# jiahuei/sparse-image-captioning

Hardware: AMD Instinct MI355X
Metric: captions/sec (higher is better)
Workload: dtype bf16; 1 GPU; configs[1]: ORT dense, 256 images x 5 captions, teacher-forcing XE fwd+bwd+clip+Adam; images_per_gpu=256, regions=36, captions_per_image=5, parallelism=single

## Files before the change

include/ortk.h:

```cpp
#ifndef ORTK_H
#define ORTK_H

#include <stddef.h>
#include <stdint.h>

#ifdef __cplusplus
extern "C" {
#endif

#define ORTK_VERSION 4
#define ORTK_EINVAL (-1)
#define ORTK_ENOSPC (-2)
#define ORTK_ENOSYS (-3)
#define ORTK_EEXCHANGE (-4)

typedef void* ortk_stream;

int ortk_version(void);
int ortk_device_ok(void);

struct ortk_sparse_plan;
typedef struct ortk_config {
    int32_t d_model, d_ff, n_layers, n_heads;
    int32_t vocab, feat, seq_len;
    int32_t pad_id, bos_id, eos_id, unk_id;
// ... 128 lines not shown
    int32_t attn16_min_lq;
    int32_t side_stream;
    int32_t row_chain;
    int32_t chain_wide;
    int32_t spmm_alias;
    int32_t f32_split;
    int32_t wgrad_wgs;
    int32_t wgrad_group;
    int32_t wgrad_group_splitk;
    int32_t wgrad_group_wgs;
    int32_t wgrad_group_tail;
    int32_t feats_bf16;
    int32_t ln_fuse;
    int32_t samp_epilogue;
    int32_t gemm_epilogue;
} ortk_tuning;
void ortk_get_tuning(ortk_tuning* out);
int ortk_set_tuning(const ortk_tuning* t);

#define ORTK_DEC_UNFUSED 1
#define ORTK_DEC_STACK 2
#define ORTK_DEC_SPARSE_STREAM 4
#define ORTK_DEC_STACK_RB20 8
#define ORTK_DEC_STACK_SPLIT 16
#define ORTK_DEC_SPLIT_SMALL 32
#define ORTK_DEC_SPARSE_GATHER 64
typedef struct ortk_decode_opts {
    int32_t beam_size;
    int32_t num_random_sample;
    float   temperature;
// ... 102 lines not shown
    float drop_p; uint32_t drop_seed;
    const float* d_o; void* dq; void* d_k; void* dv; float* dscore;
    int64_t lddo, lddq, lddk, lddv;
    int32_t o_dtype, dqkv_dtype;
    int32_t kv_dtype;
    const float* k_new; const float* v_new; int64_t ld_new;
    int32_t bwd_part;
    int32_t precision;
    int32_t qkv_dtype;
    const int32_t* q_off; int32_t q_off_stride; int32_t kv_ragged;
    int32_t drop_tf_T, drop_tf_t, drop_tf_lk;
    const int32_t* drop_rows;
} ortk_attn_args;
int ortk_attention_fwd(const ortk_attn_args* a, ortk_stream stream);
int ortk_attention_bwd(const ortk_attn_args* a, ortk_stream stream);

int ortk_embed_fwd(const int64_t* seq, int64_t seq_stride, const float* lut, const float* pe, float* out, float* keymask,
                   int64_t R, int32_t T, int32_t t0, int32_t d, int32_t pad_id, float drop_p, uint32_t seed, ortk_stream stream);
int ortk_embed_bwd(const int64_t* seq, int64_t seq_stride, const float* dout, float* dlut,
                   int64_t R, int32_t T, int32_t d, float drop_p, uint32_t seed, ortk_stream stream);

int ortk_log_softmax(float* x, int64_t rows, int32_t V, int64_t ld, float scale, ortk_stream stream);
int64_t ortk_xent_scratch_floats(int64_t rows);
int ortk_xent_fwd_bwd(const float* logits, const int64_t* targets, int64_t target_stride, int32_t T, const float* weight,
                      const float* norm_dev, float* loss_dev, float* row_loss, int64_t rows, int32_t V, int64_t ld,
                      void* dlogits, int32_t dl_dtype, int64_t ld_dl, ortk_stream stream);
int ortk_log_softmax_bwd(const float* logp, const float* dlogp, int64_t ld_in, void* dlogits, int32_t dl_dtype,
                         int64_t ld_out, int64_t rows, int32_t V, ortk_stream stream);

int ortk_colsum(const void* x, int32_t x_dtype, int64_t ld, float* out, int64_t M, int32_t N, ortk_stream stream);
// ... 39 lines not shown
```

sparse-image-captioning_amd/_lib.py:

```python
import ctypes as C
import os

import torch

_HERE = os.path.dirname(os.path.abspath(__file__))
LIB_PATH = os.path.join(_HERE, "libortk.so")


class OrtkUnavailable(RuntimeError):
    pass


class OrtkError(RuntimeError):
    pass


class Config(C.Structure):
    _fields_ = [("d_model", C.c_int32), ("d_ff", C.c_int32), ("n_layers", C.c_int32), ("n_heads", C.c_int32),
                ("vocab", C.c_int32), ("feat", C.c_int32), ("seq_len", C.c_int32),
                ("pad_id", C.c_int32), ("bos_id", C.c_int32), ("eos_id", C.c_int32), ("unk_id", C.c_int32),
                ("box_trig", C.c_int32), ("precision", C.c_int32), ("drop_src", C.c_float), ("drop", C.c_float),
                ("share_enc", C.c_int32 * 16), ("share_dec", C.c_int32 * 16),
                ("share_att_enc", C.c_int32), ("share_att_dec", C.c_int32), ("no_box", C.c_int32),
                ("sparse_fwd", C.c_void_p), ("sparse_bwd", C.c_void_p)]
# ... 57 lines not shown
                ("n2", C.c_int32), ("out2", C.c_void_p), ("drop_p", C.c_float), ("eps", C.c_float), ("drop_rows", C.c_void_p)]


class MaskedAdamArgs(C.Structure):
    _fields_ = [("w", C.c_void_p), ("g", C.c_void_p), ("mw", C.c_void_p), ("vw", C.c_void_p),
                ("ml", C.c_void_p), ("mm", C.c_void_p), ("mv", C.c_void_p),
                ("draws", C.c_void_p), ("active", C.c_void_p), ("extra_coef", C.c_void_p),
                ("n", C.c_int64), ("index0", C.c_int64), ("mode", C.c_int32), ("seed", C.c_uint32),
                ("lr_w", C.c_float), ("eps_w", C.c_float), ("lr_m", C.c_float), ("eps_m", C.c_float),
                ("beta1", C.c_float), ("beta2", C.c_float), ("clip", C.c_float), ("bc1", C.c_float), ("bc2", C.c_float)]


class Tuning(C.Structure):
    _fields_ = [("gemm_t64", C.c_int32), ("attn_impl", C.c_int32), ("attn16_min_lq", C.c_int32),
                ("side_stream", C.c_int32), ("row_chain", C.c_int32), ("chain_wide", C.c_int32), ("spmm_alias", C.c_int32), ("f32_split", C.c_int32), ("wgrad_wgs", C.c_int32),
                ("wgrad_group", C.c_int32), ("wgrad_group_splitk", C.c_int32), ("wgrad_group_wgs", C.c_int32), ("wgrad_group_tail", C.c_int32), ("feats_bf16", C.c_int32), ("ln_fuse", C.c_int32), ("samp_epilogue", C.c_int32), ("gemm_epilogue", C.c_int32)]


DEC_UNFUSED, DEC_STACK, DEC_SPARSE_STREAM, DEC_STACK_RB20, DEC_STACK_SPLIT, DEC_SPLIT_SMALL, DEC_SPARSE_GATHER = 1, 2, 4, 8, 16, 32, 64


class DecodeOpts(C.Structure):
    _fields_ = [("beam_size", C.c_int32), ("num_random_sample", C.c_int32), ("temperature", C.c_float),
                ("decoding_constraint", C.c_int32), ("length_penalty", C.c_int32), ("length_alpha", C.c_double),
                ("seed", C.c_uint64), ("sparse", C.POINTER(EllPlanStruct)), ("exec_flags", C.c_int32), ("with_greedy", C.c_int32), ("sample_row_offset", C.c_int64),
                ("train", C.c_int32), ("drop_seed", C.c_uint64), ("memory", C.c_void_p)]


class GemmArgs(C.Structure):
    _fields_ = [("A", C.c_void_p), ("B", C.c_void_p), ("C", C.c_void_p),
                ("lda", C.c_int64), ("ldb", C.c_int64), ("ldc", C.c_int64),
# ... 78 lines not shown
    "ortk_prof_enable": (_I32, [_I32]),
    "ortk_prof_collect": (_I32, [_I32, C.POINTER(_I64), C.POINTER(C.c_double), C.POINTER(C.c_double)]),
    "ortk_prof_collect_bytes": (_I32, [_I32, C.POINTER(C.c_double)]),
    "ortk_prof_collect_units": (_I32, [_I32, C.POINTER(C.c_double)]),
    "ortk_layernorm_fwd": (_I32, [_P, _P, _P, _P, _I32, _P, _I64, _I32, _F, _P]),
    "ortk_layernorm_bwd": (_I32, [_P, _P, _P, _P, _P, _P, _P, _P, _I64, _I32, _F, _P]),
    "ortk_layernorm_bwd_drop": (_I32, [_P, _P, _P, _P, _P, _P, _P, _P, _I64, _I32, _F, _P, _I32, _F, C.c_uint32, _P]),
    "ortk_layernorm_bwd_drop_rows": (_I32, [_P, _P, _P, _P, _P, _P, _P, _P, _I64, _I32, _F, _P, _I32, _F, C.c_uint32, _P, _P]),
    "ortk_layernorm_bwd_dt": (_I32, [_P, _I32, _P, _P, _P, _P, _P, _P, _P, _I64, _I32, _F, _P, _I32, _F, C.c_uint32, _P, _P]),
    "ortk_box_logbias_fwd": (_I32, [_P, C.POINTER(_P), C.POINTER(_P), C.POINTER(_F), _P, _I32, _I32, _I32, _I32, _P]),
    "ortk_box_logbias_bwd": (_I32, [_P, C.POINTER(_P), C.POINTER(_P), C.POINTER(_F), _P, C.POINTER(_P), C.POINTER(_P),
                                   _I32, _I32, _I32, _I32, _P]),
    "ortk_box_embedding": (_I32, [_P, C.POINTER(_F), _P, _I32, _I32, _P]),
    "ortk_attention_fwd": (_I32, [C.POINTER(AttnArgs), _P]),
    "ortk_attention_bwd": (_I32, [C.POINTER(AttnArgs), _P]),
    "ortk_valid_position_tables": (_I32, [_P, _I32, _I32, _P, _P, _P]),
    "ortk_embed_fwd": (_I32, [_P, _I64, _P, _P, _P, _P, _I64, _I32, _I32, _I32, _I32, _F, _U32, _P]),
    "ortk_embed_bwd": (_I32, [_P, _I64, _P, _P, _I64, _I32, _I32, _F, _U32, _P]),
    "ortk_log_softmax": (_I32, [_P, _I64, _I32, _I64, _F, _P]),
    "ortk_xent_scratch_floats": (_I64, [_I64]),
    "ortk_xent_fwd_bwd": (_I32, [_P, _P, _I64, _I32, _P, _P, _P, _P, _I64, _I32, _I64, _P, _I32, _I64, _P]),
    "ortk_log_softmax_bwd": (_I32, [_P, _P, _I64, _P, _I32, _I64, _I64, _I32, _P]),
    "ortk_colsum": (_I32, [_P, _I32, _I64, _P, _I64, _I32, _P]),
    "ortk_gate_apply": (_I32, [_P, _P, _P, _I32, _I64, _F, _P]),
    "ortk_dropout_apply": (_I32, [_P, _P, _I32, _I64, _F, _U32, _P]),
    "ortk_dropout_apply_rows": (_I32, [_P, _P, _I32, _I64, _I32, _F, _U32, _P, _P]),
    "ortk_dropout_site_seed": (_U32, [_U64, _I32, _I32, _I32]),
    "ortk_cast_bf16": (_I32, [_P, _P, _I64, _P]),
    "ortk_fill": (_I32, [_P, _I64, _F, _P]),
    "ortk_sum_scratch_floats": (_I64, [_I64]),
# ... 4 lines not shown
    "ortk_mask_bwd": (_I32, [_P, _P, _P, _P, _P, _I64, _I32, _U32, _P, _P]),
    "ortk_masked_adam_step": (_I32, [C.POINTER(MaskedAdamArgs), _P]),
    "ortk_mask_count": (_I32, [_P, _I64, _I32, _P, _P]),
    "ortk_mask_apply_draws": (_I32, [_P, _P, _P, _P, _I64, _P]),
    "ortk_mask_bwd_draws": (_I32, [_P, _P, _P, _P, _P, _P, _I64, _P, _P]),
    "ortk_decode_step_workspace_bytes": (_SZ, [_CFG, _I32]),
    "ortk_project_memory": (_I32, [_CFG, _P, _P, _I64, _P, _SZ, _P, _P]),
    "ortk_decode_step": (_I32, [_CFG, _P, _P, _I32, _I32, _I32, _I32, _P, _P, _P, _P, _I32, _P, _SZ, _P, _I64, _P]),
    "ortk_axpy_cols": (_I32, [_P, _P, _I32, _I64, _I64, _I32, _P]),
    "ortk_linear_block": (_I32, [_CFG, _I32, C.POINTER(C.c_int64), C.POINTER(C.c_int32), C.POINTER(C.c_int32)]),
    "ortk_sparse_build": (_I32, [C.POINTER(EllPlanStruct), _P, _I32, _P]),
    "ortk_spmm": (_I32, [C.POINTER(EllPlanStruct), _I32, C.POINTER(SpmmArgs), _P]),
}

_lib = None
ABI_VERSION = 4


def lib():
    global _lib
    if _lib is None:
        if not os.path.exists(LIB_PATH):
            raise OrtkUnavailable(
                f"{LIB_PATH} is missing: build it with `python -c 'import __graft_entry__ as g; g.build()'` "
                "(or `make -C sparse-image-captioning_amd/csrc`).  There is no CPU / PyTorch fallback.")
        h = C.CDLL(LIB_PATH)
        h.ortk_version.restype = C.c_int32
        if h.ortk_version() != ABI_VERSION:
            raise OrtkUnavailable(
                f"{LIB_PATH} is ABI version {h.ortk_version()}, these bindings were written for version {ABI_VERSION} (include/ortk.h: "
                "ORTK_VERSION): a stale build.  Rebuild it with `make -C sparse-image-captioning_amd/csrc`.")
# ... 52 lines not shown
```

sparse-image-captioning_amd/csrc/ortk_attn.hip:

```cpp
#include <cstdlib>
#include "ortk_internal.h"

namespace {

constexpr int MAXK = 128;
constexpr int MAXD = 64;
constexpr int KP = MAXD + 1;

__device__ __forceinline__ float bcast(float v, int l) { return __shfl(v, l, 64); }

__device__ __forceinline__ void wave_sync() { __builtin_amdgcn_fence(__ATOMIC_ACQ_REL, "wavefront"); __builtin_amdgcn_wave_barrier(); }

struct Tiles {
    float (*k)[KP];
    float (*v)[KP];
    float* mask;
    float (*q)[MAXD];
    float (*p)[MAXK];
};
__host__ __device__ inline size_t fwd_lds_bytes(int Lk) {
    return sizeof(float) * ((size_t)2 * Lk * KP + MAXK + 4 * MAXD + 4 * MAXK);
}
__device__ __forceinline__ Tiles carve_fwd(float* base, int Lk) {
    Tiles t;
// ... 1007 lines not shown
    for (int64_t i = (int64_t)blockIdx.x * 256 + threadIdx.x; i < n; i += (int64_t)gridDim.x * 256) {
        const int64_t g = i / d; const int c = (int)(i - g * d);
        const int j = a.Lk - 1;
        const int64_t row = a.kv_index ? (int64_t)a.kv_index[g * a.Lk + j] : g * (a.kv_group_stride > 0 ? a.kv_group_stride : a.Lk) + j;
        st_elem(const_cast<float*>(a.k), row * a.ldk + c, a.kv_dtype, a.k_new[g * a.ld_new + c]);
        st_elem(const_cast<float*>(a.v), row * a.ldv + c, a.kv_dtype, a.v_new[g * a.ld_new + c]);
    }
}

static bool kv16_ok(const ortk_attn_args* a) {
    const bool rowdec = a->Lq == 1 && a->H == 8 && a->dk == 64 && a->Lk <= 32 && a->causal_period == 0 && a->drop_p == 0.f && !a->bias;
    const bool small = a->dk == 64 && a->Lq <= 16 && a->Lk <= 48 && !a->kv_index && (a->Lq >= 9 || a->Lk > 8) && !rowdec;
    return (rowdec || small) && a->ldk % 8 == 0 && a->ldv % 8 == 0 && attn_impl() == 0;
}

extern "C" int ortk_attention_fwd(const ortk_attn_args* a_in, ortk_stream stream) {
    if (int e = check(a_in)) return e;
    if (!a_in->o) return ORTK_EINVAL;
    if (a_in->nkv == 0) return 0;
    if (a_in->kv_dtype != 0 && (a_in->kv_dtype != 1 || !kv16_ok(a_in))) return ORTK_EINVAL;
    ortk_attn_args a_local = *a_in;
    ortk_attn_args* a = &a_local;
    if ((a->k_new != nullptr) != (a->v_new != nullptr)) return ORTK_EINVAL;
    if (a->k_new && (a->Lq != 1 || a->ld_new < (int64_t)a->H * a->dk)) return ORTK_EINVAL;
    if (a->k_new) {
        const bool rowdec = a->H == 8 && a->dk == 64 && a->Lk <= 32 && a->causal_period == 0 && a->drop_p == 0.f && !a->bias &&
                            a->ldq % 4 == 0 && a->ldk % 4 == 0 && a->ldv % 4 == 0 && a->ldo % 4 == 0 && a->ld_new % 4 == 0 && attn_impl() == 0 &&
                            ((reinterpret_cast<uintptr_t>(a->q) | reinterpret_cast<uintptr_t>(a->k) | reinterpret_cast<uintptr_t>(a->v) |
                              reinterpret_cast<uintptr_t>(a->o) | reinterpret_cast<uintptr_t>(a->k_new) | reinterpret_cast<uintptr_t>(a->v_new)) & 15) == 0;
        if (!rowdec) {
            const int64_t n = (int64_t)a->nkv * a->H * a->dk;
            hipLaunchKernelGGL(attn_kv_append_kernel, dim3((unsigned)std::max<int64_t>(1, std::min<int64_t>(ortk_cdiv(n, 256), 2048))), dim3(256), 0,
                               ortk_s(stream), *a);
            ORTK_CHECK_LAUNCH();
            a->k_new = a->v_new = nullptr;
        }
    }
    if ((attn_impl() == 0 || a->qkv_dtype) && ortk::attn16_ok(a, false)) return ortk::attn16_fwd(a, ortk_s(stream));
    if (a->qkv_dtype || a->q_off) return ORTK_EINVAL;
    ortk::lds_attr(reinterpret_cast<const void*>(attn_fwd_kernel), fwd_lds_bytes(MAXK));
    ortk::lds_attr(reinterpret_cast<const void*>(attn_fwd_wave_kernel), sizeof(float) * 4 * (2 * 64 * KP + 128));
    if (a->drop_tf_T > 0) {
        if (a->kv_dtype || a->qkv_dtype || a->Lk > MAXK || a->dk > MAXD) return ORTK_EINVAL;
        hipLaunchKernelGGL(attn_fwd_kernel, dim3((unsigned)(a->nkv * a->H)), dim3(256), fwd_lds_bytes(a->Lk), ortk_s(stream), *a);
        ORTK_CHECK_LAUNCH();
        return 0;
    }
    const bool use_mfma = attn_impl() == 0 ? a->Lq > 32 : attn_impl() == 3;
    const bool vec_kq = (a->ldk % 4 == 0) && (a->ldq % 4 == 0) && (a->dk % 4 == 0) &&
                        ((reinterpret_cast<uintptr_t>(a->k) | reinterpret_cast<uintptr_t>(a->q)) & 15) == 0;
    const bool al16 = ((reinterpret_cast<uintptr_t>(a->q) | reinterpret_cast<uintptr_t>(a->k) | reinterpret_cast<uintptr_t>(a->v) |
                        reinterpret_cast<uintptr_t>(a->o)) & 15) == 0;
// ... 35 lines not shown
        if (DKP == 64 && Lkp == 48)      hipLaunchKernelGGL((attn_fwd_mfma_kernel<48, 64>), mgrid, mblock, lds, ortk_s(stream), *a, Lkp, DKP);
        else if (DKP == 64 && Lkp == 32) hipLaunchKernelGGL((attn_fwd_mfma_kernel<32, 64>), mgrid, mblock, lds, ortk_s(stream), *a, Lkp, DKP);
        else if (DKP == 64 && Lkp == 64) hipLaunchKernelGGL((attn_fwd_mfma_kernel<64, 64>), mgrid, mblock, lds, ortk_s(stream), *a, Lkp, DKP);
        else                             hipLaunchKernelGGL((attn_fwd_mfma_kernel<0, 0>), mgrid, mblock, lds, ortk_s(stream), *a, Lkp, DKP);
    } else if (a->Lk <= 64 && attn_impl() == 1) {
        const int pairs = a->nkv * a->H;
        hipLaunchKernelGGL(attn_fwd_wave_kernel, dim3((unsigned)ortk_cdiv(pairs, 4)), dim3(256),
                           sizeof(float) * 4 * ((size_t)2 * a->Lk * KP + 128), ortk_s(stream), *a);
    } else {
        hipLaunchKernelGGL(attn_fwd_kernel, dim3((unsigned)(a->nkv * a->H)), dim3(256), fwd_lds_bytes(a->Lk), ortk_s(stream), *a);
    }
    ORTK_CHECK_LAUNCH();
    return 0;
}

extern "C" int ortk_attention_bwd(const ortk_attn_args* a, ortk_stream stream) {
    if (int e = check(a)) return e;
    if (a->kv_dtype != 0 || a->bwd_part < 0 || a->bwd_part > 2) return ORTK_EINVAL;
    if (!a->p || !a->d_o || !a->dq || !a->d_k || !a->dv || a->kv_index || a->kv_group_stride) return ORTK_EINVAL;
    if (a->nkv == 0) return 0;
    if ((attn_impl() == 0 || a->qkv_dtype) && ortk::attn16_ok(a, true))
        return a->bwd_part == 2 ? 0 : ortk::attn16_bwd(a, ortk_s(stream));
    if (a->qkv_dtype || a->q_off) return ORTK_EINVAL;
    ortk::lds_attr(reinterpret_cast<const void*>(attn_bwd_kernel), bwd_lds_bytes(MAXK));
    ortk::lds_attr(reinterpret_cast<const void*>(attn_bwd_wave_kernel<64>), sizeof(float) * 4 * (2 * 64 * KP + 192));
    ortk::lds_attr(reinterpret_cast<const void*>(attn_bwd_wave_kernel<48>), sizeof(float) * 4 * (2 * 48 * KP + 192));
    const int pairs = a->nkv * a->H;
    if (small_ok(a) && attn_impl() == 0 && a->ldv % 4 == 0 && a->lddo % 4 == 0 &&
        ((reinterpret_cast<uintptr_t>(a->v) | reinterpret_cast<uintptr_t>(a->d_o)) & 15) == 0) {
        const dim3 sgrid((unsigned)ortk_cdiv(pairs, 4));
        const int nit = a->Lq > 16 ? 2 : 1, njt = a->Lk > 16 ? 2 : 1;
        if (nit == 2 && njt == 2)      hipLaunchKernelGGL((attn_small_bwd_kernel<2, 2>), sgrid, dim3(256), 0, ortk_s(stream), *a);
        else if (nit == 2)             hipLaunchKernelGGL((attn_small_bwd_kernel<2, 1>), sgrid, dim3(256), 0, ortk_s(stream), *a);
        else if (njt == 2)             hipLaunchKernelGGL((attn_small_bwd_kernel<1, 2>), sgrid, dim3(256), 0, ortk_s(stream), *a);
        else                           hipLaunchKernelGGL((attn_small_bwd_kernel<1, 1>), sgrid, dim3(256), 0, ortk_s(stream), *a);
// ... 45 lines not shown
```

sparse-image-captioning_amd/csrc/ortk_internal.h:

```cpp
#pragma once
#include "ortk_common.h"

namespace ortk {

const ortk_tuning& tuning();
int lds_attr(const void* fn, size_t bytes);

bool ortk_prof_active();
bool ortk_prof_serial();
constexpr int PROF_KEY_DECSTACK = 16;
constexpr int PROF_KEY_CHAIN = 17;
constexpr int PROF_KEY_WGRAD_GROUP = 18;
struct ProfMark { hipEvent_t a, b; int key; double flops, bytes; bool live; int slot = -1; double per_count = 0.0; double units = 0.0 ; };
bool prof_begin(int key, double flops, double bytes, hipStream_t s, ProfMark& m);
void prof_end(const ProfMark& m, hipStream_t s);
unsigned long long* prof_slot(int* index);

int kv_append(const float* qkv, void* cache_k, void* cache_v, int32_t kv_dtype, int64_t rows, int32_t d, int32_t row_mult, int32_t tmax,
              int32_t t, hipStream_t s);

bool attn16_shape_ok(int Lq, int Lk, int dk);
bool attn16_ok(const ortk_attn_args* a, bool bwd);
int attn16_fwd(const ortk_attn_args* a, hipStream_t s);
int attn16_bwd(const ortk_attn_args* a, hipStream_t s);

struct WBlock { int32_t off, N, K, tile0; };
constexpr int MAX_WBLOCKS = 200;
struct WBlockTable { int32_t n, tiles; WBlock b[MAX_WBLOCKS]; };
int cast_bf16_transposed(const float* x, void* yt, const WBlockTable& t, hipStream_t s);

struct BeamState {
    int32_t B, b, L, V, eos;
    int64_t ldv;
    int32_t* seq[2];
    float* tok_lp[2];
    float* cum;
    int64_t* it;
    int32_t* kvidx[2];
    int32_t* done_seq;
// ... 126 lines not shown
```

sparse-image-captioning_amd/csrc/ortk_runtime.hip:

```cpp
#include <mutex>
#include <vector>
#include "ortk_internal.h"

namespace ortk {
static ortk_tuning tuning_defaults() {
    ortk_tuning t{};
    t.gemm_t64 = 640;
    t.attn_impl = 0;
    t.attn16_min_lq = 33;
    t.side_stream = 1;
    t.row_chain = 1;
    t.chain_wide = 1;
    t.spmm_alias = 1;
    t.f32_split = 1;
    t.wgrad_wgs = 384;
    t.wgrad_group = 3;
    t.wgrad_group_splitk = 0;
    t.wgrad_group_wgs = 80;
    t.wgrad_group_tail = 1;
    t.feats_bf16 = 1;
    t.ln_fuse = 0;
    t.samp_epilogue = 1;
    t.gemm_epilogue = 0;
    return t;
}
static ortk_tuning g_tuning = tuning_defaults();
const ortk_tuning& tuning() { return g_tuning; }
}

extern "C" void ortk_get_tuning(ortk_tuning* out) { if (out) *out = ortk::g_tuning; }
extern "C" int ortk_set_tuning(const ortk_tuning* t) {
    if (!t) return ORTK_EINVAL;
    auto in = [](int32_t v, int32_t lo, int32_t hi) { return v >= lo && v <= hi; };
    if (!in(t->attn_impl, 0, 4) || t->attn16_min_lq < 1 || !in(t->f32_split, 0, 7) || t->wgrad_wgs < 1 ||
        !in(t->wgrad_group, 0, 15) || !in(t->wgrad_group_splitk, 0, 8) || t->wgrad_group_wgs < 1 || !in(t->wgrad_group_tail, 0, 1) ||
        !in(t->feats_bf16, 0, 1) || !in(t->ln_fuse, 0, 15) || (t->ln_fuse & 2)  ||
        !in(t->samp_epilogue, 0, 1) || !in(t->gemm_epilogue, 0, 3)) return ORTK_EINVAL;
    ortk::g_tuning = *t;
    return 0;
}

namespace ortk {
int lds_attr(const void* fn, size_t bytes) {
    struct Key { int dev; const void* fn; size_t bytes; };
    static std::mutex mu;
    static std::vector<Key>* seen = new std::vector<Key>();
    int dev = 0;
    if (hipGetDevice(&dev) != hipSuccess) return ORTK_EINVAL;
    std::lock_guard<std::mutex> lk(mu);
    for (const Key& k : *seen) if (k.dev == dev && k.fn == fn && k.bytes >= bytes) return 0;
    if (hipFuncSetAttribute(fn, hipFuncAttributeMaxDynamicSharedMemorySize, (int)bytes) != hipSuccess) return ORTK_EINVAL;
    seen->push_back(Key{dev, fn, bytes});
// ... 91 lines not shown
```

Measured before the change: 132,200 captions/sec.

## Add whole-row MFMA attention kernels for short ragged caption sequences

```diff
diff --git a/include/ortk.h b/include/ortk.h
--- a/include/ortk.h
+++ b/include/ortk.h
@@ -8,7 +8,7 @@
 extern "C" {
 #endif
 
-#define ORTK_VERSION 4
+#define ORTK_VERSION 5
 #define ORTK_EINVAL (-1)
 #define ORTK_ENOSPC (-2)
 #define ORTK_ENOSYS (-3)
@@ -167,6 +167,7 @@
     int32_t ln_fuse;
     int32_t samp_epilogue;
     int32_t gemm_epilogue;
+    int32_t attn_rows;
 } ortk_tuning;
 void ortk_get_tuning(ortk_tuning* out);
 int ortk_set_tuning(const ortk_tuning* t);
@@ -299,6 +300,7 @@
 } ortk_attn_args;
 int ortk_attention_fwd(const ortk_attn_args* a, ortk_stream stream);
 int ortk_attention_bwd(const ortk_attn_args* a, ortk_stream stream);
+int ortk_attention_rows_serves(const ortk_attn_args* a, int bwd);
 
 int ortk_embed_fwd(const int64_t* seq, int64_t seq_stride, const float* lut, const float* pe, float* out, float* keymask,
                    int64_t R, int32_t T, int32_t t0, int32_t d, int32_t pad_id, float drop_p, uint32_t seed, ortk_stream stream);
diff --git a/scratch/attn_rows_bench.py b/scratch/attn_rows_bench.py
--- /dev/null
+++ b/scratch/attn_rows_bench.py
@@ -0,0 +1,55 @@
+import ctypes as C, os, statistics, sys
+sys.path[:0] = [os.path.join(os.path.dirname(os.path.abspath(__file__)), "..")]
+import torch
+import sparse_image_captioning_amd as P
+L = P._lib
+vals = [int(x) for x in sys.argv[1:] if "=" not in x] or [0, 1]
+for x in sys.argv[1:]:
+    if x.startswith("lib="):
+        L.LIB_PATH = x[4:]
+lib = L.lib()
+R, T, H, dk, NSET = 1280, 17, 8, 64, 4
+d = H * dk
+g = torch.Generator().manual_seed(0)
+lens = torch.randint(2, T + 1, (R,), generator=g)
+lens[:R // 2] = T
+while int(lens.sum()) > 16640:
+    i = int(torch.randint(R // 2, R, (1,), generator=g)); lens[i] = max(2, int(lens[i]) - 1)
+while int(lens.sum()) < 16640:
+    i = int(torch.randint(R // 2, R, (1,), generator=g)); lens[i] = min(T, int(lens[i]) + 1)
+off = torch.zeros(R + 1, dtype=torch.int32); off[1:] = lens.cumsum(0)
+M = int(off[-1])
+row_pos = torch.cat([c * T + torch.arange(int(n)) for c, n in enumerate(lens)]).int()
+sets = []
+for s in range(NSET):
+    t = dict(qkv=torch.randn(M, 3 * d, device="cuda").bfloat16(), do=torch.randn(M, d, device="cuda").bfloat16(),
+             o=torch.empty(M, d, device="cuda", dtype=torch.bfloat16), p=torch.empty(R, H, T, T, device="cuda"),
+             dqkv=torch.empty(M, 3 * d, device="cuda", dtype=torch.bfloat16), km=torch.ones(M, device="cuda"), off=off.cuda(), dr=row_pos.cuda())
+    a = L.AttnArgs()
+    a.precision = a.qkv_dtype = a.o_dtype = a.dqkv_dtype = 1
+    base, dbase = t["qkv"].data_ptr(), t["dqkv"].data_ptr()
+    a.q, a.k, a.v, a.o, a.p = base, base + 2 * d, base + 4 * d, t["o"].data_ptr(), t["p"].data_ptr()
+    a.ldq = a.ldk = a.ldv = a.lddq = a.lddk = a.lddv = 3 * d
+    a.ldo = a.lddo = d
+    a.d_o, a.dq, a.d_k, a.dv = t["do"].data_ptr(), dbase, dbase + 2 * d, dbase + 4 * d
+    a.nkv, a.H, a.Lq, a.Lk, a.dk, a.causal_period = R, H, T, T, dk, T
+    a.kmask, a.q_off, a.q_off_stride, a.kv_ragged, a.drop_rows = t["km"].data_ptr(), t["off"].data_ptr(), 1, 1, t["dr"].data_ptr()
+    a.drop_p, a.drop_seed = 0.1, 11
+    sets.append((a, t))
+print(f"{R} captions, {M} rows, lib {L.LIB_PATH}", flush=True)
+for v in vals:
+    L.set_tuning(attn_rows=v)
+    line = []
+    for name, fn in (("fwd", lib.ortk_attention_fwd), ("bwd", lib.ortk_attention_bwd)):
+        for a, _ in sets:
+            L.check(fn(C.byref(a), L.stream_ptr()), name)
+        torch.cuda.synchronize()
+        for _ in range(2):
+            ev = [(torch.cuda.Event(enable_timing=True), torch.cuda.Event(enable_timing=True)) for _ in range(24)]
+            for i, (e0, e1) in enumerate(ev):
+                e0.record(); fn(C.byref(sets[i % NSET][0]), L.stream_ptr()); e1.record()
+            torch.cuda.synchronize()
+            us = [e0.elapsed_time(e1) * 1e3 for e0, e1 in ev]
+            line.append(f"{name} {min(us):6.1f} / {statistics.median(us):6.1f}")
+    serves = [lib.ortk_attention_rows_serves(C.byref(sets[0][0]), b) for b in (0, 1)] if hasattr(lib, "ortk_attention_rows_serves") else "?"
+    print(f"attn_rows {v} (whole-row kernels serve fwd, bwd: {serves}):  " + "   ".join(line), flush=True)
diff --git a/sparse-image-captioning_amd/_lib.py b/sparse-image-captioning_amd/_lib.py
--- a/sparse-image-captioning_amd/_lib.py
+++ b/sparse-image-captioning_amd/_lib.py
@@ -95,7 +95,7 @@
 class Tuning(C.Structure):
     _fields_ = [("gemm_t64", C.c_int32), ("attn_impl", C.c_int32), ("attn16_min_lq", C.c_int32),
                 ("side_stream", C.c_int32), ("row_chain", C.c_int32), ("chain_wide", C.c_int32), ("spmm_alias", C.c_int32), ("f32_split", C.c_int32), ("wgrad_wgs", C.c_int32),
-                ("wgrad_group", C.c_int32), ("wgrad_group_splitk", C.c_int32), ("wgrad_group_wgs", C.c_int32), ("wgrad_group_tail", C.c_int32), ("feats_bf16", C.c_int32), ("ln_fuse", C.c_int32), ("samp_epilogue", C.c_int32), ("gemm_epilogue", C.c_int32)]
+                ("wgrad_group", C.c_int32), ("wgrad_group_splitk", C.c_int32), ("wgrad_group_wgs", C.c_int32), ("wgrad_group_tail", C.c_int32), ("feats_bf16", C.c_int32), ("ln_fuse", C.c_int32), ("samp_epilogue", C.c_int32), ("gemm_epilogue", C.c_int32), ("attn_rows", C.c_int32)]
 
 
 DEC_UNFUSED, DEC_STACK, DEC_SPARSE_STREAM, DEC_STACK_RB20, DEC_STACK_SPLIT, DEC_SPLIT_SMALL, DEC_SPARSE_GATHER = 1, 2, 4, 8, 16, 32, 64
@@ -204,6 +204,7 @@
     "ortk_box_embedding": (_I32, [_P, C.POINTER(_F), _P, _I32, _I32, _P]),
     "ortk_attention_fwd": (_I32, [C.POINTER(AttnArgs), _P]),
     "ortk_attention_bwd": (_I32, [C.POINTER(AttnArgs), _P]),
+    "ortk_attention_rows_serves": (_I32, [C.POINTER(AttnArgs), _I32]),
     "ortk_valid_position_tables": (_I32, [_P, _I32, _I32, _P, _P, _P]),
     "ortk_embed_fwd": (_I32, [_P, _I64, _P, _P, _P, _P, _I64, _I32, _I32, _I32, _I32, _F, _U32, _P]),
     "ortk_embed_bwd": (_I32, [_P, _I64, _P, _P, _I64, _I32, _I32, _F, _U32, _P]),
@@ -238,7 +239,7 @@
 }
 
 _lib = None
-ABI_VERSION = 4
+ABI_VERSION = 5
 
 
 def lib():
diff --git a/sparse-image-captioning_amd/csrc/ortk_attn.hip b/sparse-image-captioning_amd/csrc/ortk_attn.hip
--- a/sparse-image-captioning_amd/csrc/ortk_attn.hip
+++ b/sparse-image-captioning_amd/csrc/ortk_attn.hip
@@ -1045,6 +1045,8 @@
     return (rowdec || small) && a->ldk % 8 == 0 && a->ldv % 8 == 0 && attn_impl() == 0;
 }
 
+static bool rows_serves(const ortk_attn_args* a, bool bwd) { return (attn_impl() == 0 || a->qkv_dtype) && ortk::attn_rows_ok(a, bwd); }
+
 extern "C" int ortk_attention_fwd(const ortk_attn_args* a_in, ortk_stream stream) {
     if (int e = check(a_in)) return e;
     if (!a_in->o) return ORTK_EINVAL;
@@ -1067,6 +1069,7 @@
             a->k_new = a->v_new = nullptr;
         }
     }
+    if (rows_serves(a, false)) return ortk::attn_rows_fwd(a, ortk_s(stream));
     if ((attn_impl() == 0 || a->qkv_dtype) && ortk::attn16_ok(a, false)) return ortk::attn16_fwd(a, ortk_s(stream));
     if (a->qkv_dtype || a->q_off) return ORTK_EINVAL;
     ortk::lds_attr(reinterpret_cast<const void*>(attn_fwd_kernel), fwd_lds_bytes(MAXK));
@@ -1132,11 +1135,24 @@
     return 0;
 }
 
-extern "C" int ortk_attention_bwd(const ortk_attn_args* a, ortk_stream stream) {
+static int check_bwd(const ortk_attn_args* a) {
     if (int e = check(a)) return e;
     if (a->kv_dtype != 0 || a->bwd_part < 0 || a->bwd_part > 2) return ORTK_EINVAL;
     if (!a->p || !a->d_o || !a->dq || !a->d_k || !a->dv || a->kv_index || a->kv_group_stride) return ORTK_EINVAL;
+    return 0;
+}
+
+extern "C" int ortk_attention_rows_serves(const ortk_attn_args* a, int bwd) {
+    if (int e = bwd ? check_bwd(a) : check(a)) return e;
+    if (!bwd && !a->o) return ORTK_EINVAL;
+    return a->nkv > 0 && rows_serves(a, bwd != 0) ? 1 : 0;
+}
+
+extern "C" int ortk_attention_bwd(const ortk_attn_args* a, ortk_stream stream) {
+    if (int e = check_bwd(a)) return e;
     if (a->nkv == 0) return 0;
+    if (rows_serves(a, true))
+        return a->bwd_part == 2 ? 0 : ortk::attn_rows_bwd(a, ortk_s(stream));
     if ((attn_impl() == 0 || a->qkv_dtype) && ortk::attn16_ok(a, true))
         return a->bwd_part == 2 ? 0 : ortk::attn16_bwd(a, ortk_s(stream));
     if (a->qkv_dtype || a->q_off) return ORTK_EINVAL;
diff --git a/sparse-image-captioning_amd/csrc/ortk_attn_rows.hip b/sparse-image-captioning_amd/csrc/ortk_attn_rows.hip
--- /dev/null
+++ b/sparse-image-captioning_amd/csrc/ortk_attn_rows.hip
@@ -0,0 +1,439 @@
+#include <cstdlib>
+#include "ortk_internal.h"
+
+namespace {
+
+constexpr int PJ = 40;
+
+__device__ __forceinline__ void wsync() { __builtin_amdgcn_fence(__ATOMIC_ACQ_REL, "wavefront"); __builtin_amdgcn_wave_barrier(); }
+__device__ __forceinline__ bf16x4 cvt4(float4 v) { return (bf16x4){(__bf16)v.x, (__bf16)v.y, (__bf16)v.z, (__bf16)v.w}; }
+__device__ __forceinline__ bf16x4 cvt4(f32x4 v) { return (bf16x4){(__bf16)v[0], (__bf16)v[1], (__bf16)v[2], (__bf16)v[3]}; }
+__device__ __forceinline__ f32x4 mma(bf16x8 x, bf16x8 y, f32x4 acc) { return __builtin_amdgcn_mfma_f32_16x16x32_bf16(x, y, acc, 0, 0, 0); }
+
+template <int PITCH>
+__device__ __forceinline__ bf16x8 frag_row(const __bf16* img, int row, int k0) {
+    return *reinterpret_cast<const bf16x8*>(img + row * PITCH + k0);
+}
+template <int PITCH>
+__device__ __forceinline__ bf16x8 frag_tr(const __bf16* img, int x0, int lane, int zr) {
+    const int lr = lane & 15, lq = lane >> 4;
+    const int r0 = 8 * lq + (lr >> 2);
+    const int c = x0 + 4 * (lane & 3);
+    typedef bf16x4 __attribute__((address_space(3))) * lds4;
+    const bf16x4 lo = __builtin_amdgcn_ds_read_tr16_b64_v4bf16((lds4)(img + min(r0, zr) * PITCH + c));
+    const bf16x4 hi = __builtin_amdgcn_ds_read_tr16_b64_v4bf16((lds4)(img + min(r0 + 4, zr) * PITCH + c));
+    return (bf16x8){lo[0], lo[1], lo[2], lo[3], hi[0], hi[1], hi[2], hi[3]};
+}
+
+template <int DKT, int HW, int NU>
+__device__ __forceinline__ void span_load(bf16x8 (&v)[NU], const __bf16* src, int64_t ld, int rows, int nh, int tid) {
+    constexpr int CPH = DKT / 8, CPR = HW * CPH, NT = 64 * HW;
+#pragma unroll
+    for (int u = 0; u < NU; ++u) {
+        const int idx = tid + u * NT, r = idx / CPR, c = idx % CPR;
+        v[u] = (bf16x8){0, 0, 0, 0, 0, 0, 0, 0};
+        if (r < rows && c < nh * CPH) v[u] = *reinterpret_cast<const bf16x8*>(src + (int64_t)r * ld + c * 8);
+    }
+}
+template <int DKT, int HW, int NU>
+__device__ __forceinline__ void span_store(const bf16x8 (&v)[NU], __bf16* img, int rows_img, int tid) {
+    constexpr int CPH = DKT / 8, CPR = HW * CPH, NT = 64 * HW, PD = DKT + 8;
+#pragma unroll
+    for (int u = 0; u < NU; ++u) {
+        const int idx = tid + u * NT, r = idx / CPR, c = idx % CPR;
+        if (r < rows_img) *reinterpret_cast<bf16x8*>(img + ((c / CPH) * rows_img + r) * PD + (c % CPH) * 8) = v[u];
+    }
+}
+template <int DKT, int HW>
+__device__ __forceinline__ void span_out(__bf16* dst, int64_t ld, const __bf16* img, int rows_img, int rows, int nh, int tid) {
+    constexpr int CPH = DKT / 8, CPR = HW * CPH, NT = 64 * HW, PD = DKT + 8;
+    for (int idx = tid; idx < rows * CPR; idx += NT) {
+        const int r = idx / CPR, c = idx % CPR;
+        if (c < nh * CPH)
+            *reinterpret_cast<bf16x8*>(dst + (int64_t)r * ld + c * 8) = *reinterpret_cast<const bf16x8*>(img + ((c / CPH) * rows_img + r) * PD + (c % CPH) * 8);
+    }
+}
+
+__device__ __forceinline__ int step_rem(int rem, int r, int LL, int& carry) {
+    rem += r; carry = 0;
+    if (LL >= 4) { if (rem >= LL) { rem -= LL; carry = 1; } }
+    else { carry = rem / LL; rem -= carry * LL; }
+    return rem;
+}
+
+struct Geo { int64_t row0; int n; };
+__device__ __forceinline__ Geo group_rows(const ortk_attn_args& a, int g, int L) {
+    Geo o;
+    o.row0 = a.q_off ? (int64_t)a.q_off[(int64_t)g * a.q_off_stride] : (int64_t)g * L;
+    o.n = a.q_off ? min(L, (int)(a.q_off[(int64_t)(g + 1) * a.q_off_stride] - o.row0)) : L;
+    return o;
+}
+
+template <int NT, int DKT, int HW>
+__global__ __launch_bounds__(64 * HW) void attn_rows_fwd_kernel(ortk_attn_args a) {
+    constexpr int DK = DKT, PD = DKT + 8, NU = NT == 1 ? 3 : 5;
+    const float qscale = DKT == 64 ? 0.125f : 0.17677669529663687f;
+    extern __shared__ __attribute__((aligned(16))) unsigned char sm_rows[];
+    const int tid = threadIdx.x, lane = tid & 63, wave = tid >> 6;
+    const int lr = lane & 15, lq = lane >> 4;
+    const int L = a.Lq, LL = L * L;
+    const int nhb = (a.H + HW - 1) / HW;
+    const int g = blockIdx.x / nhb, h0 = (blockIdx.x - g * nhb) * HW, nh = min(HW, a.H - h0), h = h0 + wave;
+    const Geo grp = group_rows(a, g, L);
+    const int Lg = grp.n;
+    float* sPf = reinterpret_cast<float*>(sm_rows);
+    float* sMask = sPf + ((HW * LL + 3) & ~3);
+    __bf16* sQ = reinterpret_cast<__bf16*>(sMask + 32);
+    __bf16* sK = sQ + HW * L * PD;
+    __bf16* sV = sK + HW * L * PD;
+    __bf16* sP = sV + HW * (L + 1) * PD + wave * 16 * PJ;
+    bf16x8 vq[NU], vk[NU], vv[NU];
+    span_load<DK, HW, NU>(vq, reinterpret_cast<const __bf16*>(a.q) + grp.row0 * a.ldq + h0 * DK, a.ldq, Lg, nh, tid);
+    span_load<DK, HW, NU>(vk, reinterpret_cast<const __bf16*>(a.k) + grp.row0 * a.ldk + h0 * DK, a.ldk, Lg, nh, tid);
+    span_load<DK, HW, NU>(vv, reinterpret_cast<const __bf16*>(a.v) + grp.row0 * a.ldv + h0 * DK, a.ldv, Lg, nh, tid);
+    float mk_in = -1.f;
+    if (tid < 32 && tid < Lg) mk_in = a.kmask ? a.kmask[grp.row0 + tid] : 1.f;
+    int di[NT];
+#pragma unroll
+    for (int it = 0; it < NT; ++it) {
+        const int i = 16 * it + lr;
+        di[it] = i;
+        if (a.drop_rows && a.q_off && a.drop_p > 0.f && i < Lg) di[it] = (int)((int64_t)a.drop_rows[grp.row0 + i] - (int64_t)g * L);
+    }
+    span_store<DK, HW, NU>(vq, sQ, L, tid);
+    span_store<DK, HW, NU>(vk, sK, L, tid);
+    span_store<DK, HW, NU>(vv, sV, L + 1, tid);
+    if (tid < 32) sMask[tid] = mk_in;
+    if (NT == 1)
+        for (int idx = lane; idx < 16 * 8; idx += 64) *reinterpret_cast<bf16x4*>(sP + (idx >> 3) * PJ + (idx & 7) * 4) = cvt4(make_float4(0.f, 0.f, 0.f, 0.f));
+    __syncthreads();
+    const float inv_keep = a.drop_p > 0.f ? 1.f / (1.f - a.drop_p) : 1.f;
+    if (wave < nh) {
+        __bf16* sQh = sQ + wave * L * PD;
+        const __bf16* sKh = sK + wave * L * PD;
+        const __bf16* sVh = sV + wave * (L + 1) * PD;
+        float* sPh = sPf + wave * LL;
+        bf16x8 qf[NT][DK / 32];
+#pragma unroll
+        for (int it = 0; it < NT; ++it)
+#pragma unroll
+            for (int ks = 0; ks < DK / 32; ++ks) qf[it][ks] = frag_row<PD>(sQh, min(16 * it + lr, L - 1), 32 * ks + 8 * lq);
+#pragma unroll
+        for (int it = 0; it < NT; ++it) {
+            if (16 * it >= Lg) break;
+            const int i = 16 * it + lr;
+            const bool iv = i < Lg;
+            const int64_t drow = (((int64_t)g * a.H + h) * L + di[it]) * L;
+            f32x4 s[NT];
+#pragma unroll
+            for (int jt = 0; jt < NT; ++jt) {
+                s[jt] = (f32x4){0.f, 0.f, 0.f, 0.f};
+#pragma unroll
+                for (int ks = 0; ks < DK / 32; ++ks) s[jt] = mma(frag_row<PD>(sKh, min(16 * jt + lr, L - 1), 32 * ks + 8 * lq), qf[it][ks], s[jt]);
+            }
+            const int qpos = a.causal_period > 0 ? i % a.causal_period : 0;
+            float mx = -INFINITY;
+#pragma unroll
+            for (int jt = 0; jt < NT; ++jt) {
+                const int j0 = 16 * jt + 4 * lq;
+#pragma unroll
+                for (int r = 0; r < 4; ++r) {
+                    const int j = j0 + r;
+                    const float mk = sMask[j];
+                    float x = s[jt][r] * qscale;
+                    if (mk == 0.f || (a.causal_period > 0 && j > qpos)) x = -1e9f;
+                    if (mk < 0.f) x = -INFINITY;
+                    s[jt][r] = x;
+                    mx = fmaxf(mx, x);
+                }
+            }
+            mx = fmaxf(mx, __shfl_xor(mx, 16, 64)); mx = fmaxf(mx, __shfl_xor(mx, 32, 64));
+            float sum = 0.f;
+#pragma unroll
+            for (int jt = 0; jt < NT; ++jt)
+#pragma unroll
+                for (int r = 0; r < 4; ++r) { const float e = expf(s[jt][r] - mx); s[jt][r] = e; sum += e; }
+            sum += __shfl_xor(sum, 16, 64); sum += __shfl_xor(sum, 32, 64);
+#pragma unroll
+            for (int jt = 0; jt < NT; ++jt) {
+                const int j0 = 16 * jt + 4 * lq;
+                float p[4];
+#pragma unroll
+                for (int r = 0; r < 4; ++r) p[r] = (iv && j0 + r < L) ? s[jt][r] / sum : 0.f;
+                if (a.p && iv) {
+#pragma unroll
+                    for (int r = 0; r < 4; ++r) if (j0 + r < L) sPh[i * L + j0 + r] = p[r];
+                }
+                if (a.drop_p > 0.f) {
+                    bool kp[4];
+                    ortk_keep4(a.drop_seed, (uint64_t)(drow + j0), a.drop_p, kp);
+#pragma unroll
+                    for (int r = 0; r < 4; ++r) p[r] = kp[r] ? p[r] * inv_keep : 0.f;
+                }
+                *reinterpret_cast<bf16x4*>(sP + lr * PJ + j0) = cvt4(make_float4(p[0], p[1], p[2], p[3]));
+            }
+            wsync();
+            const bf16x8 pf = frag_row<PJ>(sP, lr, 8 * lq);
+#pragma unroll
+            for (int dt = 0; dt < DK / 16; ++dt) {
+                const f32x4 o = mma(frag_tr<PD>(sVh, 16 * dt, lane, L), pf, (f32x4){0.f, 0.f, 0.f, 0.f});
+                if (iv) {
+                    if (a.o_dtype == ORTK_BF16) *reinterpret_cast<bf16x4*>(sQh + i * PD + 16 * dt + 4 * lq) = cvt4(o);
+                    else st_elem4(a.o, (grp.row0 + i) * a.ldo + h * DK + 16 * dt + 4 * lq, ORTK_F32, make_float4(o[0], o[1], o[2], o[3]));
+                }
+            }
+            wsync();
+        }
+    }
+    __syncthreads();
+    if (a.o_dtype == ORTK_BF16)
+        span_out<DK, HW>(reinterpret_cast<__bf16*>(a.o) + grp.row0 * a.ldo + h0 * DK, a.ldo, sQ, L, Lg, nh, tid);
+    if (a.p) {
+        const int n = nh * LL, lim = Lg * L;
+        const int64_t base = ((int64_t)g * a.H + h0) * LL;
+        float* gp = a.p + base;
+        const bool vec = (base & 3) == 0;
+        const int sr = (4 * 64 * HW) % LL;
+        int rem0 = (4 * tid) % LL, carry;
+        for (int e0 = 4 * tid; e0 < n; e0 += 4 * 64 * HW) {
+            if (vec && rem0 + 3 < lim) {
+                *reinterpret_cast<float4*>(gp + e0) = *reinterpret_cast<const float4*>(sPf + e0);
+            } else {
+                for (int r = 0; r < 4 && e0 + r < n; ++r) if (step_rem(rem0, r, LL, carry) < lim) gp[e0 + r] = sPf[e0 + r];
+            }
+            rem0 = step_rem(rem0, sr, LL, carry);
+        }
+    }
+}
+
+template <int NT, int DKT, int HW>
+__global__ __launch_bounds__(64 * HW) void attn_rows_bwd_kernel(ortk_attn_args a) {
+    constexpr int DK = DKT, PD = DKT + 8, NU = NT == 1 ? 3 : 5, NUP = NT == 1 ? 1 : 4, NDT = DK / 16;
+    const float qscale = DKT == 64 ? 0.125f : 0.17677669529663687f;
+    extern __shared__ __attribute__((aligned(16))) unsigned char sm_rows[];
+    const int tid = threadIdx.x, lane = tid & 63, wave = tid >> 6;
+    const int lr = lane & 15, lq = lane >> 4;
+    const int L = a.Lq, LL = L * L;
+    const int nhb = (a.H + HW - 1) / HW;
+    const int g = blockIdx.x / nhb, h0 = (blockIdx.x - g * nhb) * HW, nh = min(HW, a.H - h0), h = h0 + wave;
+    const Geo grp = group_rows(a, g, L);
+    const int Lg = grp.n;
+    const int SDH = 2 * (L + 1) * PJ;
+    __bf16* sK = reinterpret_cast<__bf16*>(sm_rows);
+    __bf16* sV = sK + HW * (L + 1) * PD;
+    __bf16* sQ = sV + HW * L * PD;
+    __bf16* sG = sQ + HW * (L + 1) * PD;
+    __bf16* sSD = sG + HW * (L + 1) * PD;
+    bf16x8 vk[NU], vv[NU], vq[NU], vg[NU];
+    span_load<DK, HW, NU>(vk, reinterpret_cast<const __bf16*>(a.k) + grp.row0 * a.ldk + h0 * DK, a.ldk, Lg, nh, tid);
+    span_load<DK, HW, NU>(vv, reinterpret_cast<const __bf16*>(a.v) + grp.row0 * a.ldv + h0 * DK, a.ldv, Lg, nh, tid);
+    span_load<DK, HW, NU>(vq, reinterpret_cast<const __bf16*>(a.q) + grp.row0 * a.ldq + h0 * DK, a.ldq, Lg, nh, tid);
+    span_load<DK, HW, NU>(vg, reinterpret_cast<const __bf16*>(a.d_o) + grp.row0 * a.lddo + h0 * DK, a.lddo, Lg, nh, tid);
+    const int n = nh * LL, lim = Lg * L;
+    const int64_t base = ((int64_t)g * a.H + h0) * LL;
+    const float* gp = a.p + base;
+    const bool vec = (base & 3) == 0;
+    float4 vp[NUP];
+    int ph[NUP], pr[NUP], carry;
+    ph[0] = (4 * tid) / LL; pr[0] = 4 * tid - ph[0] * LL;
+#pragma unroll
+    for (int u = 1; u < NUP; ++u) {
+        const int sh = (4 * 64 * HW) / LL, sr = 4 * 64 * HW - sh * LL;
+        pr[u] = step_rem(pr[u - 1], sr, LL, carry); ph[u] = ph[u - 1] + sh + carry;
+    }
+#pragma unroll
+    for (int u = 0; u < NUP; ++u) {
+        const int e0 = 4 * (tid + u * 64 * HW);
+        vp[u] = make_float4(0.f, 0.f, 0.f, 0.f);
+        if (vec && e0 + 3 < n && pr[u] + 3 < lim) vp[u] = *reinterpret_cast<const float4*>(gp + e0);
+        else if (e0 < n) { float* q = &vp[u].x; for (int r = 0; r < 4; ++r) if (e0 + r < n && step_rem(pr[u], r, LL, carry) < lim) q[r] = gp[e0 + r]; }
+    }
+    int di[NT];
+#pragma unroll
+    for (int it = 0; it < NT; ++it) {
+        const int i = 16 * it + lr;
+        di[it] = i;
+        if (a.drop_rows && a.q_off && a.drop_p > 0.f && i < Lg) di[it] = (int)((int64_t)a.drop_rows[grp.row0 + i] - (int64_t)g * L);
+    }
+    span_store<DK, HW, NU>(vk, sK, L + 1, tid);
+    span_store<DK, HW, NU>(vv, sV, L, tid);
+    span_store<DK, HW, NU>(vq, sQ, L + 1, tid);
+    span_store<DK, HW, NU>(vg, sG, L + 1, tid);
+#pragma unroll
+    for (int u = 0; u < NUP; ++u) {
+        const int e0 = 4 * (tid + u * 64 * HW);
+        const float* q = &vp[u].x;
+#pragma unroll
+        for (int r = 0; r < 4; ++r) {
+            const int rem = step_rem(pr[u], r, LL, carry);
+            if (e0 + r < n) reinterpret_cast<float*>(sSD + (ph[u] + carry) * SDH)[rem] = q[r];
+        }
+    }
+    __syncthreads();
+    const float inv_keep = a.drop_p > 0.f ? 1.f / (1.f - a.drop_p) : 1.f;
+    if (wave < nh) {
+        __bf16* sKh = sK + wave * (L + 1) * PD;
+        __bf16* sVh = sV + wave * L * PD;
+        __bf16* sQh = sQ + wave * (L + 1) * PD;
+        const __bf16* sGh = sG + wave * (L + 1) * PD;
+        __bf16* sS = sSD + wave * SDH;
+        __bf16* sD = sS + (L + 1) * PJ;
+        float4 praw[NT][NT];
+        {
+            const float* sPh = reinterpret_cast<const float*>(sS);
+#pragma unroll
+            for (int it = 0; it < NT; ++it)
+#pragma unroll
+                for (int jt = 0; jt < NT; ++jt) {
+                    const int i = 16 * it + lr, j0 = 16 * jt + 4 * lq;
+                    float* q = &praw[it][jt].x;
+#pragma unroll
+                    for (int r = 0; r < 4; ++r) q[r] = (i < Lg && j0 + r < L) ? sPh[i * L + j0 + r] : 0.f;
+                }
+        }
+        wsync();
+        for (int idx = lane; idx < SDH / 4; idx += 64) *reinterpret_cast<bf16x4*>(sS + idx * 4) = cvt4(make_float4(0.f, 0.f, 0.f, 0.f));
+        wsync();
+#pragma unroll
+        for (int it = 0; it < NT; ++it) {
+            if (16 * it >= Lg) break;
+            const int i = 16 * it + lr;
+            const bool iv = i < Lg;
+            const int64_t drow = (((int64_t)g * a.H + h) * L + di[it]) * L;
+            bf16x8 gf[DK / 32];
+#pragma unroll
+            for (int ks = 0; ks < DK / 32; ++ks) gf[ks] = frag_row<PD>(sGh, min(i, L), 32 * ks + 8 * lq);
+            f32x4 dp[NT], pp[NT];
+            float dot = 0.f;
+#pragma unroll
+            for (int jt = 0; jt < NT; ++jt) {
+                dp[jt] = (f32x4){0.f, 0.f, 0.f, 0.f};
+#pragma unroll
+                for (int ks = 0; ks < DK / 32; ++ks) dp[jt] = mma(frag_row<PD>(sVh, min(16 * jt + lr, L - 1), 32 * ks + 8 * lq), gf[ks], dp[jt]);
+                const int j0 = 16 * jt + 4 * lq;
+                const float pv[4] = {praw[it][jt].x, praw[it][jt].y, praw[it][jt].z, praw[it][jt].w};
+                float pd[4];
+                bool kp[4] = {true, true, true, true};
+                if (a.drop_p > 0.f) ortk_keep4(a.drop_seed, (uint64_t)(drow + j0), a.drop_p, kp);
+#pragma unroll
+                for (int r = 0; r < 4; ++r) {
+                    const bool valid = iv && j0 + r < L;
+                    const bool keep = valid && kp[r];
+                    const float d = keep ? dp[jt][r] * inv_keep : 0.f;
+                    pd[r] = keep ? pv[r] * inv_keep : 0.f;
+                    pp[jt][r] = valid ? pv[r] : 0.f; dp[jt][r] = d; dot += pp[jt][r] * d;
+                }
+                if (i < L) *reinterpret_cast<bf16x4*>(sD + i * PJ + j0) = cvt4(make_float4(pd[0], pd[1], pd[2], pd[3]));
+            }
+            dot += __shfl_xor(dot, 16, 64); dot += __shfl_xor(dot, 32, 64);
+#pragma unroll
+            for (int jt = 0; jt < NT; ++jt) {
+                const int j0 = 16 * jt + 4 * lq;
+                float ds[4];
+#pragma unroll
+                for (int r = 0; r < 4; ++r) ds[r] = pp[jt][r] * (dp[jt][r] - dot);
+                if (i < L) *reinterpret_cast<bf16x4*>(sS + i * PJ + j0) = cvt4(make_float4(ds[0] * qscale, ds[1] * qscale, ds[2] * qscale, ds[3] * qscale));
+            }
+        }
+        wsync();
+#pragma unroll
+        for (int it = 0; it < NT; ++it) {
+            if (16 * it >= Lg) break;
+            const int i = 16 * it + lr;
+            const bool iv = i < Lg;
+            const bf16x8 sf = frag_row<PJ>(sS, min(i, L), 8 * lq);
+#pragma unroll
+            for (int dt = 0; dt < NDT; ++dt) {
+                const f32x4 acc = mma(frag_tr<PD>(sKh, 16 * dt, lane, L), sf, (f32x4){0.f, 0.f, 0.f, 0.f});
+                if (iv) {
+                    if (a.dqkv_dtype == ORTK_BF16) *reinterpret_cast<bf16x4*>(sVh + i * PD + 16 * dt + 4 * lq) = cvt4(acc);
+                    else st_elem4(a.dq, (grp.row0 + i) * a.lddq + h * DK + 16 * dt + 4 * lq, ORTK_F32, make_float4(acc[0], acc[1], acc[2], acc[3]));
+                }
+            }
+        }
+        wsync();
+#pragma unroll
+        for (int which = 0; which < 2; ++which) {
+            const __bf16* sA = which == 0 ? sS : sD;
+            const __bf16* sB = which == 0 ? sQh : sGh;
+            __bf16* sO = which == 0 ? sKh : sQh;
+#pragma unroll
+            for (int jt = 0; jt < NT; ++jt) {
+                if (16 * jt >= Lg) break;
+                const bf16x8 af = frag_tr<PJ>(sA, 16 * jt, lane, L);
+                const int j = 16 * jt + lr;
+#pragma unroll
+                for (int dt = 0; dt < NDT; ++dt) {
+                    const f32x4 acc = mma(frag_tr<PD>(sB, 16 * dt, lane, L), af, (f32x4){0.f, 0.f, 0.f, 0.f});
+                    if (j < Lg) {
+                        if (a.dqkv_dtype == ORTK_BF16) *reinterpret_cast<bf16x4*>(sO + j * PD + 16 * dt + 4 * lq) = cvt4(acc);
+                        else st_elem4(which == 0 ? a.d_k : a.dv, (grp.row0 + j) * (which == 0 ? a.lddk : a.lddv) + h * DK + 16 * dt + 4 * lq, ORTK_F32,
+                                      make_float4(acc[0], acc[1], acc[2], acc[3]));
+                    }
+                }
+            }
+            wsync();
+        }
+    }
+    __syncthreads();
+    if (a.dqkv_dtype == ORTK_BF16) {
+        span_out<DK, HW>(reinterpret_cast<__bf16*>(a.dq) + grp.row0 * a.lddq + h0 * DK, a.lddq, sV, L, Lg, nh, tid);
+        span_out<DK, HW>(reinterpret_cast<__bf16*>(a.d_k) + grp.row0 * a.lddk + h0 * DK, a.lddk, sK, L + 1, Lg, nh, tid);
+        span_out<DK, HW>(reinterpret_cast<__bf16*>(a.dv) + grp.row0 * a.lddv + h0 * DK, a.lddv, sQ, L + 1, Lg, nh, tid);
+    }
+}
+
+size_t fwd_rows_lds(int L, int dk, int hw) {
+    return (size_t)((hw * L * L + 3) & ~3) * sizeof(float) + 32 * sizeof(float) +
+           ((size_t)hw * (3 * L + 1) * (dk + 8) + (size_t)hw * 16 * PJ) * sizeof(__bf16);
+}
+size_t bwd_rows_lds(int L, int dk, int hw) {
+    return ((size_t)hw * (4 * L + 3) * (dk + 8) + (size_t)hw * 2 * (L + 1) * PJ) * sizeof(__bf16);
+}
+bool al16(const void* p) { return (reinterpret_cast<uintptr_t>(p) & 15) == 0; }
+
+constexpr int HW = 4;
+typedef void (*rows_fn)(ortk_attn_args);
+rows_fn pick_rows(bool bwd, int nt, int dk) {
+    if (bwd) {
+        if (dk == 64) return nt == 1 ? attn_rows_bwd_kernel<1, 64, HW> : attn_rows_bwd_kernel<2, 64, HW>;
+        return nt == 1 ? attn_rows_bwd_kernel<1, 32, HW> : attn_rows_bwd_kernel<2, 32, HW>;
+    }
+    if (dk == 64) return nt == 1 ? attn_rows_fwd_kernel<1, 64, HW> : attn_rows_fwd_kernel<2, 64, HW>;
+    return nt == 1 ? attn_rows_fwd_kernel<1, 32, HW> : attn_rows_fwd_kernel<2, 32, HW>;
+}
+
+int launch_rows(const ortk_attn_args* a, bool bwd, hipStream_t s) {
+    const int L = a->Lq, nt = L > 16 ? 2 : 1;
+    const size_t lds = bwd ? bwd_rows_lds(L, a->dk, HW) : fwd_rows_lds(L, a->dk, HW);
+    const rows_fn fn = pick_rows(bwd, nt, a->dk);
+    if (lds > 64 * 1024) ortk::lds_attr(reinterpret_cast<const void*>(fn), 160 * 1024);
+    hipLaunchKernelGGL(fn, dim3((unsigned)((int64_t)a->nkv * ((a->H + HW - 1) / HW))), dim3(64 * HW), lds, s, *a);
+    ORTK_CHECK_LAUNCH();
+    return 0;
+}
+
+}
+
+namespace ortk {
+
+bool attn_rows_ok(const ortk_attn_args* a, bool bwd) {
+    if (!tuning().attn_rows || a->precision != 1 || a->qkv_dtype != 1) return false;
+    if (a->Lq != a->Lk || a->Lq < 1 || a->Lq > 32 || (a->dk != 64 && a->dk != 32) || a->H < 1) return false;
+    if (a->bias || a->kv_index || a->kv_group_stride > 0 || a->kv_dtype != 0 || a->k_new || a->v_new || a->drop_tf_T > 0) return false;
+    if (a->q_off && (a->kv_ragged != 1 || a->q_off_stride < 1)) return false;
+    if ((a->ldq | a->ldk | a->ldv) % 8 || !al16(a->q) || !al16(a->k) || !al16(a->v)) return false;
+    if (!bwd) {
+        if (a->ldo % (a->o_dtype == ORTK_BF16 ? 8 : 4) || !al16(a->o) || (a->p && !al16(a->p))) return false;
+    } else {
+        if (!a->p || !a->d_o || !a->dq || !a->d_k || !a->dv || a->dscore) return false;
+        if (a->lddo % 8 || (a->lddq | a->lddk | a->lddv) % (a->dqkv_dtype == ORTK_BF16 ? 8 : 4)) return false;
+        if (!al16(a->d_o) || !al16(a->p) || !al16(a->dq) || !al16(a->d_k) || !al16(a->dv)) return false;
+    }
+    return true;
+}
+
+int attn_rows_fwd(const ortk_attn_args* a, hipStream_t s) { return launch_rows(a, false, s); }
+int attn_rows_bwd(const ortk_attn_args* a, hipStream_t s) { return launch_rows(a, true, s); }
+
+}
diff --git a/sparse-image-captioning_amd/csrc/ortk_internal.h b/sparse-image-captioning_amd/csrc/ortk_internal.h
--- a/sparse-image-captioning_amd/csrc/ortk_internal.h
+++ b/sparse-image-captioning_amd/csrc/ortk_internal.h
@@ -23,6 +23,9 @@
 bool attn16_ok(const ortk_attn_args* a, bool bwd);
 int attn16_fwd(const ortk_attn_args* a, hipStream_t s);
 int attn16_bwd(const ortk_attn_args* a, hipStream_t s);
+bool attn_rows_ok(const ortk_attn_args* a, bool bwd);
+int attn_rows_fwd(const ortk_attn_args* a, hipStream_t s);
+int attn_rows_bwd(const ortk_attn_args* a, hipStream_t s);
 
 struct WBlock { int32_t off, N, K, tile0; };
 constexpr int MAX_WBLOCKS = 200;
diff --git a/sparse-image-captioning_amd/csrc/ortk_runtime.hip b/sparse-image-captioning_amd/csrc/ortk_runtime.hip
--- a/sparse-image-captioning_amd/csrc/ortk_runtime.hip
+++ b/sparse-image-captioning_amd/csrc/ortk_runtime.hip
@@ -22,6 +22,7 @@
     t.ln_fuse = 0;
     t.samp_epilogue = 1;
     t.gemm_epilogue = 0;
+    t.attn_rows = 1;
     return t;
 }
 static ortk_tuning g_tuning = tuning_defaults();
@@ -35,7 +36,8 @@
     if (!in(t->attn_impl, 0, 4) || t->attn16_min_lq < 1 || !in(t->f32_split, 0, 7) || t->wgrad_wgs < 1 ||
         !in(t->wgrad_group, 0, 15) || !in(t->wgrad_group_splitk, 0, 8) || t->wgrad_group_wgs < 1 || !in(t->wgrad_group_tail, 0, 1) ||
         !in(t->feats_bf16, 0, 1) || !in(t->ln_fuse, 0, 15) || (t->ln_fuse & 2)  ||
-        !in(t->samp_epilogue, 0, 1) || !in(t->gemm_epilogue, 0, 3)) return ORTK_EINVAL;
+        !in(t->samp_epilogue, 0, 1) || !in(t->gemm_epilogue, 0, 3) ||
+        !in(t->attn_rows, 0, 1)) return ORTK_EINVAL;
     ortk::g_tuning = *t;
     return 0;
 }
```

New measurement: 133,700 captions/sec, median of 6. +1.2%, better.
